# google/forma

Hardware: AMD Instinct MI355X
Metric: frames/sec (sorted+painted, device-resident) + Mpixel-segments/sec (higher is better)
Workload: dtype u64 segments / f64+f32 rasterizer / f32 painter; 1 GPU; paris-like-30k-4k (labelled stand-in: paris-30k.svg is not in the reference checkout); layers=30000, pixel_segments=13757174, frames_in_flight=3

## Files before the change

forma_amd/csrc/api.cpp:

```cpp
#include <new>

#include "ctx.h"

#ifndef FORMA_ARCH
#define FORMA_ARCH "gfx950"
#endif

thread_local KernelTimer* g_ktimer = nullptr;
static inline float* kt_us(forma_hip_ctx* c) { return c->kt_dur_us; }

int fd_fail(forma_hip_ctx* c, int code, const char* what, hipError_t e) {
    if (c) snprintf(c->err, sizeof c->err, "%s%s%s", what, e != hipSuccess ? ": " : "", e != hipSuccess ? hipGetErrorString(e) : "");
    return code;
}

namespace {

inline int fail(forma_hip_ctx* c, int code, const char* what, hipError_t e = hipSuccess) { return fd_fail(c, code, what, e); }
void share_scene(forma_hip_ctx* o);
void invalidate_counts(forma_hip_ctx* o);
inline forma_hip_ctx* last_slot(forma_hip_ctx* ctx) { return ctx->last ? ctx->last : ctx; }
#define HIPCHECK(expr)                                                        \
    do {                                                                      \
        hipError_t _e = (expr);                                               \
// ... 52 lines not shown
    const uint32_t bf_cap = (uint32_t)std::min<size_t>(ctx->block_first.cap / 4, 0xFFFFFFFFu);
    stage_begin(ctx, ST_PREPARE, timing);
    launch_prepare_compact(ctx->stream, src, (uint32_t)n_lines, ctx->cl_idx.as<uint32_t>(), ctx->cl_start.as<uint32_t>(),
                           ctx->block_first.as<uint32_t>(), bf_cap, ctx->prep_scratch.as<uint32_t>(), ctx->info.as<FrameInfo>(), zero);
    stage_end(ctx, ST_PREPARE, timing);
    HIPCHECK(hipGetLastError());
    if (bound_n) return FORMA_OK;
    int rc = read_info(ctx);
    if (rc) return rc;
    const size_t N = ctx->h_info->n_segments;
    ctx->n_seg = N; ctx->n_compact = ctx->h_info->n_compact;
    const size_t need = (N + RAS_TILE - 1) / RAS_TILE + 1;
    if (need > bf_cap) {
        HIPCHECK(ctx->block_first.ensure(need * 4 * 2));
        launch_block_first(ctx->stream, ctx->cl_start.as<uint32_t>(), (uint32_t)ctx->n_compact, (uint32_t)N,
                           ctx->block_first.as<uint32_t>());
    }
    return FORMA_OK;
}

LineSource geometry_source(forma_hip_ctx* ctx, uint32_t width, uint32_t height) {
    LineSource S;
    memset(&S, 0, sizeof S);
    const size_t l0 = ctx->line_ranged ? ctx->line_lo : 0;
    S.x = ctx->x.as<float>() + l0; S.y = ctx->y.as<float>() + l0; S.line_slot = ctx->line_slot.as<uint32_t>() + l0;
    S.geoms = ctx->geoms.as<forma_geom_t>(); S.n_geoms = (uint32_t)ctx->n_geoms;
    S.width = (float)width; S.height = (float)height;
    S.band_lo = -3.0e38f; S.band_hi = 3.0e38f;
    if (ctx->band_row1 > 0) { S.band_lo = (float)(ctx->band_row0 * 16u) - 0.125f; S.band_hi = (float)(ctx->band_row1 * 16u) + 0.125f; }
    return S;
}

int finish_rasterize(forma_hip_ctx* ctx) {
    int rc = read_info(ctx);
    if (rc) return rc;
    uint64_t k_or = (uint64_t)ctx->h_info->key_or | ((uint64_t)ctx->h_info->key_or_hi << 32);
    uint64_t k_and = (uint64_t)ctx->h_info->key_and | ((uint64_t)ctx->h_info->key_and_hi << 32);
    ctx->live44 = (k_or ^ k_and) & 0xFFFFFFFFFFFull;
    ctx->layer_sorted = ctx->h_info->layer_unsorted == 0;
    return FORMA_OK;
}

SortPlan frame_sort_plan(forma_hip_ctx* ctx, uint64_t live44, bool layer_sorted, int digit_bits, bool speculated, bool* biased);
static bool fuse_plan_ok(const forma_hip_ctx* ctx, const SortPlan& plan);

int run_rasterize_frame(forma_hip_ctx* ctx, uint32_t width, uint32_t height, bool timing, bool speculate = false,
                        uint32_t bound_n = 0, const ZeroJobs* zero = nullptr, const forma_hip_ctx::PreZero* cleared = nullptr,
                        bool hist_too = false ) {
    const size_t all_lines = ctx->n_points ? ctx->n_points - 1 : 0;
    const size_t n_lines = ctx->line_ranged ? std::min(ctx->line_hi, all_lines) - std::min(ctx->line_lo, all_lines) : all_lines;
    ctx->n_lines = n_lines;
    ctx->n_seg = 0; ctx->n_compact = 0; ctx->have_unsorted = true; ctx->live44 = 0; ctx->layer_sorted = true;
    ctx->speculated = false; ctx->ras_hist_on = false; ctx->ras_fused = false;
    ctx->pz = forma_hip_ctx::PreZero();
    int rc = reset_info(ctx);
    if (rc) return rc;
    if (n_lines == 0) return FORMA_OK;
    const LineSource S = geometry_source(ctx, width, height);
    if ((rc = run_line_table(ctx, S, n_lines, timing, bound_n, zero))) return rc;
    if (zero && cleared) ctx->pz = *cleared;
    FrameInfo* dinfo = ctx->info.as<FrameInfo>();
    DevCount nc_seg, nc_cmp;
    if (bound_n) {
        nc_seg = DevCount{&dinfo->n_segments, bound_n};
        nc_cmp = DevCount{&dinfo->n_compact, (uint32_t)n_lines};
    } else {
        const size_t N = ctx->n_seg;
        if (N == 0) return FORMA_OK;
        if (N >= (1ull << 30)) return fail(ctx, FORMA_E_CAPACITY, "more than 2^30-1 pixel segments on one device");
        nc_seg = DevCount{nullptr, (uint32_t)N};
        nc_cmp = DevCount{nullptr, (uint32_t)ctx->n_compact};
    }
    HIPCHECK(ctx->seg_u.ensure(((size_t)nc_seg.bound + SEG_PAD) * 8));
    HIPCHECK(ctx->ras_masks.ensure(((size_t)nc_seg.bound / RAS_TILE + 2) * 32));
    RasHist RH;
    memset(&RH, 0, sizeof RH);
    if (hist_too && bound_n && ctx->pred_valid && ctx->pz.sort_p && ctx->pz.sort_p == ctx->sort_counters.p && !ctx->dbg.no_ras_hist) {
        ctx->ras_plan = frame_sort_plan(ctx, ctx->pred_live44, ctx->pred_layer_sorted, ctx->digit_bits, true, nullptr);
        RH = make_ras_hist(ctx->ras_plan, ctx->sort_counters.as<uint32_t>());
        ctx->ras_hist_on = RH.hist != nullptr;
        if (RH.hist && ctx->pz.slice_p && ctx->pz.slice_p == ctx->slice_buf.p && ctx->pz.slice_words >= slice_tab_words(bound_n) &&
            fuse_plan_ok(ctx, ctx->ras_plan)) {
            const SliceSrc SS = make_slice_src(ctx->slice_buf.as<uint32_t>(), bound_n);
            RH.slice_tab = SS.tab; RH.tab_stride = SS.tab_stride;
            ctx->ras_fused = true;
        }
        {
            const SortPlan plain = make_segment_sort_plan(ctx->pred_live44, ctx->pred_layer_sorted, ctx->digit_bits, nullptr, nullptr);
            const SortPlan lay = ctx->pred_layer_sorted ? SortPlan{} : make_sort_plan((ctx->pred_live44 & 0x1FFFFFull) << 20, 20, 41, ctx->digit_bits);
            bool biased = false;
            for (int p = 0; p < ctx->ras_plan.n_passes; p++) biased |= ctx->ras_plan.fmask[p] != 0u;
            RH.track_range = (biased || plain.n_passes > (ctx->pred_layer_sorted ? 0 : lay.n_passes) + 2) ? 1u : 0u;
        }
    }
    stage_begin(ctx, ST_RASTER, timing);
    launch_rasterize(ctx->stream, S, nc_cmp, nc_seg, ctx->cl_idx.as<uint32_t>(), ctx->cl_start.as<uint32_t>(),
                     ctx->block_first.as<uint32_t>(), ctx->seg_u.as<uint64_t>(), dinfo, (int)ctx->band_row0,
                     (int)ctx->band_row1, ctx->ras_masks.as<uint32_t>(), bound_n == 0, &RH);
    ctx->pending_masks = bound_n ? PendingMasks{ctx->ras_masks.as<uint32_t>(), 0u, ctx->ras_hist_on ? 1u : 0u} : PendingMasks{nullptr, 0u, 0u};
    ctx->seg_u_fused = ctx->ras_fused; ctx->fused_w = width; ctx->fused_h = height;
    stage_end(ctx, ST_RASTER, timing);
    HIPCHECK(hipGetLastError());
    ctx->speculated = (speculate || bound_n) && ctx->pred_valid;
    if (ctx->speculated) {
        ctx->live44 = ctx->pred_live44; ctx->layer_sorted = ctx->pred_layer_sorted;
        return FORMA_OK;
    }
    return finish_rasterize(ctx);
}

static uint32_t sort_workgroups(const forma_hip_ctx* ctx, size_t n_keys) {
    if (ctx->dbg.sort_cus >= 0) return (uint32_t)ctx->dbg.sort_cus;
    const forma_hip_ctx* o = ctx->owner ? ctx->owner : ctx;
    const size_t slots = o->slots.size();
    if (ctx->frame_has_dst) return 0u;
    return slots == 3 || (slots == 2 && n_keys >= ((size_t)1 << 22)) ? o->n_cus / 2u : 0u;
}

#ifndef CARRY_HALF_SLICED
#define CARRY_HALF_SLICED 1
#endif
static bool one_frame_in_flight(const forma_hip_ctx* ctx) {
    const forma_hip_ctx* o = ctx->owner ? ctx->owner : ctx;
    return o->slots.size() <= 1;
}
static bool paint_by_strips(const forma_hip_ctx* ctx, uint32_t tiles_painted) {
    if (ctx->dbg.strip_tiles >= 0) return tiles_painted <= (uint32_t)ctx->dbg.strip_tiles;
    return tiles_painted <= paint_strip_tiles(ctx) && !ctx->scene_simple && (uint64_t)ctx->costly_layers * 32u >= ctx->n_orders && one_frame_in_flight(ctx);
}

static bool paint_by_quads(const forma_hip_ctx* ctx, int cache_id, uint32_t runs_bound, uint32_t tiles) {
    if (!ctx->scene_simple || ctx->dbg.no_simple_paint || cache_id >= 0 || ctx->dbg.paint_quad == 0) return false;
    if (ctx->dbg.paint_quad == 2) return true;
    return tiles >= 16u * 8192u && (uint64_t)runs_bound <= 8ull * tiles;
}

static void ban_bias(forma_hip_ctx* ctx) {
    ctx->bias_ban_len = ctx->bias_ban_len ? std::min(ctx->bias_ban_len * 2u, 4096u) : 64u;
    ctx->bias_banned = ctx->bias_ban_len;
}

SortPlan frame_sort_plan(forma_hip_ctx* ctx, uint64_t live44, bool layer_sorted, int digit_bits, bool speculated, bool* biased) {
    const KeyRange* range = speculated && ctx->pred_range.valid && !ctx->bias_banned && !ctx->dbg.no_bias ? &ctx->pred_range : nullptr;
    return make_segment_sort_plan(live44, layer_sorted, digit_bits, range, biased);
}

#ifndef FUSE_MIN_SLICE
#define FUSE_MIN_SLICE 28
#endif
#ifndef FUSE_PROBE
#define FUSE_PROBE 256
#endif
static bool fuse_plan_ok(const forma_hip_ctx* ctx, const SortPlan& plan) {
    if (ctx->dbg.fuse_digit == 0 || ctx->dbg.no_ras_hist || ctx->digit_bits == 4) return false;
    if (ctx->band_row1 > 0 || ctx->line_ranged) return false;
    return plan.n_passes >= 2 && plan.n_passes <= RH_MAX_PASSES && plan.mask[0] <= 255u;
}
static bool fuse_first_digit(forma_hip_ctx* ctx, const SortPlan& plan) {
    if (!fuse_plan_ok(ctx, plan)) return false;
    if (ctx->dbg.fuse_digit == 2 || ctx->pred_slice_len == 0 || ctx->pred_slice_len >= FUSE_MIN_SLICE) return true;
    if (++ctx->fuse_skipped < FUSE_PROBE) return false;
    ctx->fuse_skipped = 0;
    return true;
}

int plan_zero_jobs(forma_hip_ctx* ctx, uint32_t width, uint32_t height, uint32_t sort_n, uint32_t runs_n, ZeroJobs* Z,
                   forma_hip_ctx::PreZero* cleared) {
// ... 1947 lines not shown
```

forma_amd/csrc/common.h:

```cpp
#pragma once
#include <hip/hip_runtime.h>
#include <hip/hip_ext.h>
#include <stdint.h>
#include <stddef.h>

#include "../../include/forma_hip.h"

#define SEG_KEY_SHIFT 20
#define SEG_KEY_BITS  44

#if defined(__HIPCC__)
#define FD __device__ __forceinline__
#else
#define FD inline
#endif

FD int      seg_tile_y(uint64_t v) { return (int)(v >> 53) - 1; }
FD int      seg_tile_x(uint64_t v) { return (int)((v >> 41) & 0xFFFu) - 1; }
FD uint32_t seg_layer(uint64_t v) { return (uint32_t)(v >> 20) & 0x1FFFFFu; }
FD int      seg_lx(uint64_t v) { return (int)(v >> 16) & 0xF; }
FD int      seg_ly(uint64_t v) { return (int)(v >> 12) & 0xF; }
FD int      seg_dam(uint64_t v) { return (int)(v >> 6) & 0x3F; }
FD int      seg_cover(uint64_t v) { return ((int)(v & 0x3F) ^ 0x20) - 0x20; }
FD uint64_t seg_key(uint64_t v) { return v >> SEG_KEY_SHIFT; }
// ... 63 lines not shown
    uint4*   list;
    uint32_t cap;
    uint32_t min_row;
};

struct TileCacheArgs {
    uint2*         tiles;
    uint8_t*       written;
};
#define REF_SPAN 0x80000000u
#define REF_UNCH 0x40000000u
#define REF_IDX  0x3FFFFFFFu

struct DevCount {
    const uint32_t* ptr;
    uint32_t bound;
};
#if defined(__HIPCC__)
__device__ __forceinline__ uint32_t dev_count(DevCount c) { return c.ptr ? min(*c.ptr, c.bound) : c.bound; }
#endif

struct KernelTimer {
    static constexpr int CAP = 96;
    hipEvent_t e0[CAP], e1[CAP];
    const char* name[CAP];
    int stage[CAP];
    int n = 0, made = 0, cur_stage = 0;
    int dropped = 0;
    hipStream_t stream = nullptr;
};
extern thread_local KernelTimer* g_ktimer;
inline bool ktimer_slot(KernelTimer* kt, const char* name, hipEvent_t* e0, hipEvent_t* e1) {
    if (!kt) return false;
    if (kt->n >= KernelTimer::CAP) { kt->dropped++; return false; }
    if (kt->n >= kt->made) {
        if (hipEventCreate(&kt->e0[kt->made]) != hipSuccess) return false;
        if (hipEventCreate(&kt->e1[kt->made]) != hipSuccess) { (void)hipEventDestroy(kt->e0[kt->made]); return false; }
        kt->made++;
    }
    const int i = kt->n++;
    kt->name[i] = name; kt->stage[i] = kt->cur_stage;
    *e0 = kt->e0[i]; *e1 = kt->e1[i];
    return true;
}
#define FORMA_LAUNCH(kern, grid, block, shm, s, ...)                                                        \
    do {                                                                                                    \
        hipEvent_t fl_e0_, fl_e1_;                                                                          \
        if (g_ktimer && g_ktimer->stream == (s) && ktimer_slot(g_ktimer, #kern, &fl_e0_, &fl_e1_))          \
            hipExtLaunchKernelGGL(kern, grid, block, shm, s, fl_e0_, fl_e1_, 0, __VA_ARGS__);               \
        else                                                                                                \
            hipLaunchKernelGGL(kern, grid, block, shm, s, __VA_ARGS__);                                     \
    } while (0)

void launch_prepare_lines(hipStream_t s, const float* x, const float* y, const uint32_t* line_slot, uint32_t n_lines,
                          const forma_geom_t* geoms, uint32_t n_geoms, float width, float height, float band_lo,
                          float band_hi, uint32_t* orders, float* x0, float* y0, float* dx, float* dy, float* a,
                          float* b, float* c, float* d, uint32_t* lengths);
size_t scan_tmp_words(size_t n);
void launch_inclusive_scan_u32(hipStream_t s, uint32_t* data, size_t n, uint32_t* tmp, uint32_t* d_total);
void launch_exclusive_scan_u32(hipStream_t s, uint32_t* data, size_t n, uint32_t* tmp, uint32_t* d_total);
void launch_scan_small_u32(hipStream_t s, uint32_t* data, DevCount n, uint32_t per, uint32_t* d_total);

#define RAS_TILE 2048u
struct PendingMasks { const uint32_t* rec; uint32_t n_fixed; uint32_t has_range; };
struct LineSource {
    const float* x; const float* y; const uint32_t* line_slot; const forma_geom_t* geoms; uint32_t n_geoms;
    float width, height, band_lo, band_hi;
    const uint32_t* sums;
    const uint32_t* orders; const float *x0, *y0, *dx, *dy, *a, *b, *c, *d;
};
size_t prepare_scratch_words(size_t n_lines);
struct ZeroJobs;
void launch_prepare_compact(hipStream_t s, const LineSource& src, uint32_t n_lines, uint32_t* cl_idx, uint32_t* cl_start,
                            uint32_t* block_first, uint32_t bf_cap, uint32_t* scratch, FrameInfo* info,
                            const ZeroJobs* zero );
void launch_line_lengths(hipStream_t s, const LineSource& src, uint32_t n_lines, uint32_t* lens, uint32_t* scratch );
void launch_block_first(hipStream_t s, const uint32_t* cl_start, uint32_t n_compact, uint32_t n_segments,
                        uint32_t* block_first);
#define HS_COPIES  16
#define SORT_BINS  512
#define RH_MAX_PASSES 3
struct RasHist { uint32_t* hist; uint32_t n_passes; uint32_t shift[RH_MAX_PASSES], mask[RH_MAX_PASSES], bias[RH_MAX_PASSES], fmask[RH_MAX_PASSES];
                 uint32_t track_range;
                 uint32_t* slice_tab; uint32_t tab_stride;  };
void launch_rasterize(hipStream_t s, const LineSource& src, DevCount n_compact, DevCount n_segments,
                      const uint32_t* cl_idx, const uint32_t* cl_start, const uint32_t* block_first, uint64_t* out,
                      FrameInfo* info, int band_row0, int band_row1, uint32_t* wg_masks ,
                      bool reduce_now ,
                      const RasHist* hist = nullptr);
void launch_flatten(hipStream_t s, const forma_flatten_tables_t* dev_tables, float* out_x, float* out_y);

#define SORT_MAX_PASSES 12
struct SortPlan {
    int      n_passes;
    int      shift[SORT_MAX_PASSES];
    uint32_t mask[SORT_MAX_PASSES];
    uint32_t bias[SORT_MAX_PASSES];
    uint32_t fmask[SORT_MAX_PASSES];
};
struct KeyRange { uint32_t min_x, max_x, min_y, max_y; bool valid; };
SortPlan make_sort_plan(uint64_t live_mask, int lo_bit, int hi_bit, int digit_bits);
SortPlan make_segment_sort_plan(uint64_t live44, bool layer_sorted, int digit_bits, const KeyRange* range, bool* biased);
size_t sort_scratch_words(size_t n);
size_t sort_zero_words(size_t n, const SortPlan& plan);
const uint32_t* sort_range_words(const uint32_t* scratch);
struct SliceSrc {
    uint32_t* tab; uint32_t tab_stride; uint32_t* first; uint32_t first_cap; uint2* ent; uint32_t ent_cap; };
struct ChunkedSrc { const uint64_t* buckets; uint32_t n_chunks; uint32_t capacity; uint32_t* mask_records; };
uint32_t sort_hist_blocks(size_t n);
const uint64_t* launch_radix_sort(hipStream_t s, const uint64_t* in, uint64_t* a, uint64_t* b, DevCount n,
                                  const SortPlan& plan, int digit_bits, uint32_t* scratch, uint32_t* err,
                                  const ChunkedSrc* chunked = nullptr, FrameInfo* info = nullptr,
                                  bool scratch_is_zero = false ,
                                  bool hist_ready = false ,
                                  uint32_t max_workgroups = 0 ,
                                  const SliceSrc* sliced = nullptr );
RasHist make_ras_hist(const SortPlan& plan, uint32_t* sort_scratch);
#define SLICE_NZ_ROW (SORT_MAX_PASSES - 1)
size_t slice_scratch_words(size_t n);
size_t slice_tab_words(size_t n);
SliceSrc make_slice_src(uint32_t* scratch, size_t n);

#define FORMA_MAX_RANKS 8
struct OwnerBands { uint32_t n; uint32_t edge[FORMA_MAX_RANKS + 1]; };
size_t owner_scratch_words(size_t n);
void launch_owner_bucket(hipStream_t s, const uint64_t* seg, DevCount n, const OwnerBands& B, uint32_t capacity,
                         uint32_t* scratch, uint64_t* send, FrameInfo* info);
void launch_row_histogram(hipStream_t s, const uint64_t* seg, DevCount n, uint32_t* hist );
size_t gather_mask_words(uint32_t n_ranks, uint32_t capacity);
void launch_gather_chunks(hipStream_t s, const uint64_t* recv, uint32_t n_ranks, uint32_t capacity,
                          uint64_t* out, FrameInfo* info, uint32_t* mask_records , bool reduce_now);

struct BlkEdge {
    uint32_t cov[4];
    uint32_t cnt;
    uint32_t has_boundary;
    uint32_t pad[2];
};
size_t runs_scratch_words(size_t n);
size_t runs_blocks(size_t n);
struct RunStyle {
    const uint32_t* layer_sf;
    uint32_t        n_orders;
    const uint8_t*  unchanged;
    uint32_t*       run_lt;
};
#define RUN_LT_OPEN 0x8000u
#define RUN_LT_NEWTILE 0x4000u
struct BlkRuns {
    const TileRecord* rec_sp;
    const uint32_t*   run_lt_sp;
    const uint32_t*   heads;
    const uint32_t*   row_sp;
    uint32_t*         row_base_out;
    uint32_t*         tile_first_run;
    uint32_t*         run_lt_out;
    uint32_t          round_tiles;
};
void launch_runs(hipStream_t s, const uint64_t* sorted, DevCount n, uint32_t tiles_w, uint32_t tiles_h, TileRecord* records,
                 uint32_t rec_cap, uint64_t* run_keys, uint32_t* tile_first_run, BlkEdge* blk_edge,
                 uint32_t* row_tab, uint32_t* scratch, FrameInfo* info, bool verify_plan, uint64_t spec_live44,
                 bool spec_layer_sorted, PendingMasks pm, RunStyle rs, bool tables_are_zero,
                 const uint32_t* range_records ,
                 uint32_t n_range_records ,
                 int what = 3 ,
                 uint32_t* chain_row_base = nullptr ,
                 bool chain_status_is_zero = false ,
// ... 90 lines not shown
```

forma_amd/csrc/debug.h:

```cpp
#pragma once
#include <cstdlib>
#include <cstring>
#include <algorithm>

struct ForMaDebug {
    bool sync = false, global_runsort = false, xgather = false, no_small_carry = false, span_groups = false, no_span_groups = false;
    bool no_packed_copy = false, no_simple_paint = false, force_simple_paint = false, trim_debug = false, force_exchange = false;
    bool xchg_copy = false, no_prezero = false, no_bias = false, no_ras_hist = false, no_cull = false, force_cull = false, no_order = false;
    int carry_slices = 0, digit_bits = 0, poison = -1, poison_frame = -1, strip_tiles = -1, carry_half = 1, paint_quad = 1, order_thr = -1, sort_cus = -1, runs_chain = -1, multi_layout = 0, carry_covl = 1, runs_blk = -1, blk_round = 256, tail_poll = 1, paint_split = 1, split_first = 25, fuse_digit = 1;
};

inline ForMaDebug forma_debug_parse() {
    ForMaDebug d;
    const char* e = getenv("FORMA_HIP_DEBUG");
    if (!e) return d;
    char buf[512];
    strncpy(buf, e, sizeof buf - 1); buf[sizeof buf - 1] = 0;
    char* save = nullptr;
    for (char* tok = strtok_r(buf, ",; ", &save); tok; tok = strtok_r(nullptr, ",; ", &save)) {
        char* val = strchr(tok, '=');
        if (val) *val++ = 0;
        const long v = val ? strtol(val, nullptr, 0) : 0;
#define FD_FLAG(name) if (!strcmp(tok, #name)) { d.name = true; continue; }
        FD_FLAG(sync) FD_FLAG(global_runsort) FD_FLAG(xgather) FD_FLAG(no_small_carry) FD_FLAG(span_groups) FD_FLAG(no_span_groups)
        FD_FLAG(no_cull) FD_FLAG(force_cull) FD_FLAG(no_order) FD_FLAG(no_prezero) FD_FLAG(no_bias) FD_FLAG(no_ras_hist) FD_FLAG(no_packed_copy) FD_FLAG(no_simple_paint) FD_FLAG(force_simple_paint) FD_FLAG(trim_debug) FD_FLAG(force_exchange)
#undef FD_FLAG
        if (!strcmp(tok, "xchg")) { d.xchg_copy = val && !strcmp(val, "copy"); continue; }
        if (!strcmp(tok, "multi_layout")) { d.multi_layout = val && !strcmp(val, "exchange") ? 1 : (val && !strcmp(val, "bands") ? 2 : 0); continue; }
        if (!strcmp(tok, "carry_slices")) { d.carry_slices = (int)v; continue; }
        if (!strcmp(tok, "digit_bits")) { d.digit_bits = (int)v; continue; }
        if (!strcmp(tok, "carry_half")) { d.carry_half = (int)std::max(v, 0L); continue; }
        if (!strcmp(tok, "carry_covl")) { d.carry_covl = (int)std::max(v, 0L); continue; }
        if (!strcmp(tok, "sort_cus")) { d.sort_cus = (int)std::max(v, 0L); continue; }
        if (!strcmp(tok, "order_thr")) { d.order_thr = (int)std::max(v, 0L); continue; }
        if (!strcmp(tok, "paint_quad")) { d.paint_quad = (int)std::max(v, 0L); continue; }
        if (!strcmp(tok, "runs_chain")) { d.runs_chain = (int)std::max(v, 0L); continue; }
        if (!strcmp(tok, "runs_blk")) { d.runs_blk = (int)std::max(v, 0L); continue; }
        if (!strcmp(tok, "blk_round")) { d.blk_round = (int)std::min(std::max(v, 1L), 256L); continue; }
        if (!strcmp(tok, "paint_split")) { d.paint_split = (int)std::min(std::max(v, 0L), 8L); continue; }
        if (!strcmp(tok, "split_first")) { d.split_first = (int)std::min(std::max(v, 1L), 99L); continue; }
        if (!strcmp(tok, "fuse_digit")) { d.fuse_digit = (int)std::min(std::max(v, 0L), 2L); continue; }
        if (!strcmp(tok, "tail_poll")) { d.tail_poll = (int)std::max(v, 0L); continue; }
        if (!strcmp(tok, "strip_tiles")) { d.strip_tiles = (int)std::max(v, 0L); continue; }
        if (!strcmp(tok, "poison")) { d.poison = (int)(v & 0xFF); continue; }
        if (!strcmp(tok, "poison_frame")) { d.poison_frame = (int)(v & 0xFF); continue; }
    }
    return d;
}
```

forma_amd/csrc/lines.hip:

```cpp
#include "common.h"
#include "lookback.h"
#include "radix_rank.h"
#include <string.h>
#ifdef RAS_PROF
__device__ unsigned long long g_ras_prof[64][8];
#define RP_STAMP(i) do { const unsigned long long _t = __builtin_readcyclecounter(); if (threadIdx.x == 0) atomicAdd(&g_ras_prof[blockIdx.x & 63][i], _t - rp_t); rp_t = __builtin_readcyclecounter(); } while (0)
extern "C" int forma_hip_debug_ras_prof(unsigned long long* out8, int reset) {
    static unsigned long long h[64][8];
    if (reset) { for (int c = 0; c < 64; c++) for (int i = 0; i < 8; i++) h[c][i] = 0; return (int)hipMemcpyToSymbol(HIP_SYMBOL(g_ras_prof), h, sizeof h); }
    int rc = (int)hipMemcpyFromSymbol(h, HIP_SYMBOL(g_ras_prof), sizeof h);
    for (int i = 0; i < 8; i++) { out8[i] = 0; for (int c = 0; c < 64; c++) out8[i] += h[c][i]; }
    return rc;
}
#else
#define RP_STAMP(i) do { } while (0)
#endif

#define WAVE 64

__device__ __forceinline__ uint32_t wave_inclusive_scan(uint32_t v) {
    const int lane = threadIdx.x & 63;
#pragma unroll
    for (int d = 1; d < 64; d <<= 1) {
        uint32_t t = __shfl_up(v, d, 64);
// ... 416 lines not shown
}

__device__ __forceinline__ uint64_t rasterize_one(uint32_t order, float lx0, float ly0, float ldx, float ldy, float a,
                                                  float b, float c, float d, double a_ab, double b_ab, double cd_ab,
                                                  uint32_t seg_i) {
    int i = (int)seg_i - (c != 0.0f ? 1 : 0) - (d != 0.0f ? 1 : 0);
    float t0 = fmaxf(find_term(i, a_ab, b_ab, cd_ab, a, b, c, d), 0.0f);
    float t1 = fminf(find_term(i + 1, a_ab, b_ab, cd_ab, a, b, c, d), 1.0f);
    float x0f = fmaf(t0, ldx, lx0), y0f = fmaf(t0, ldy, ly0);
    float x1f = fmaf(t1, ldx, lx0), y1f = fmaf(t1, ldy, ly0);
    int x0s = (int)floorf(x0f + 0.5f), x1s = (int)floorf(x1f + 0.5f);
    int y0s = (int)floorf(y0f + 0.5f), y1s = (int)floorf(y1f + 0.5f);
    int border_x = min(x0s, x1s) >> 4, border_y = min(y0s, y1s) >> 4;
    int tile_x = (int)(int16_t)(border_x >> 4), tile_y = (int)(int16_t)(border_y >> 4);
    uint32_t lx = (uint32_t)border_x & 15u, ly = (uint32_t)border_y & 15u;
    int border = (int)((uint32_t)border_x << 4) + 16;
    uint32_t dam = (uint32_t)(abs(x1s - x0s) + 2 * (border - max(x0s, x1s))) & 0xFFu;
    int cover = (int)(int8_t)(y1s - y0s);
    int ty1 = (int)(int16_t)(tile_y + 1), tx1 = (int)(int16_t)(tile_x + 1);
    uint64_t v = (uint64_t)(ty1 > 0 ? ty1 : 0) & 0x7FFull;
    v = (v << 12) | ((uint64_t)(tx1 > 0 ? tx1 : 0) & 0xFFFull);
    v = (v << 21) | ((uint64_t)order & 0x1FFFFFull);
    v = (v << 4) | lx;
    v = (v << 4) | ly;
    v = (v << 6) | (dam & 0x3Fu);
    v = (v << 6) | ((uint32_t)cover & 0x3Fu);
    return v;
}

__device__ __forceinline__ int round_half_up(float x) { return (int)floorf(x + 0.5f); }
__device__ __forceinline__ float find_term_k(int i, double a_k, double b_k, double cda_k, double cdb_k, float a, float b, float c, float d) {
    const float fi = (float)i;
    const float ja = (float)ceil(fma(b_k, (double)fi, cdb_k));
    const float jb = (float)ceil(fma(a_k, (double)fi, cda_k));
    return fminf(fmaf(a, ja, c), fmaf(b, jb, d));
}
__device__ __forceinline__ uint64_t rasterize_one_k(uint32_t order, float lx0, float ly0, float ldx, float ldy, float a, float b, float c,
                                                    float d, double a_k, double b_k, double cda_k, double cdb_k, int i) {
    float t0 = fmaxf(find_term_k(i, a_k, b_k, cda_k, cdb_k, a, b, c, d), 0.0f);
    float t1 = fminf(find_term_k(i + 1, a_k, b_k, cda_k, cdb_k, a, b, c, d), 1.0f);
    float x0f = fmaf(t0, ldx, lx0), y0f = fmaf(t0, ldy, ly0);
    float x1f = fmaf(t1, ldx, lx0), y1f = fmaf(t1, ldy, ly0);
    int x0s = round_half_up(x0f), x1s = round_half_up(x1f);
    int y0s = round_half_up(y0f), y1s = round_half_up(y1f);
    int border_x = min(x0s, x1s) >> 4, border_y = min(y0s, y1s) >> 4;
    int tile_x = (int)(int16_t)(border_x >> 4), tile_y = (int)(int16_t)(border_y >> 4);
    uint32_t lx = (uint32_t)border_x & 15u, ly = (uint32_t)border_y & 15u;
    int border = (int)((uint32_t)border_x << 4) + 16;
    uint32_t dam = (uint32_t)(abs(x1s - x0s) + 2 * (border - max(x0s, x1s))) & 0xFFu;
    int cover = (int)(int8_t)(y1s - y0s);
    int ty1 = (int)(int16_t)(tile_y + 1), tx1 = (int)(int16_t)(tile_x + 1);
    uint64_t v = (uint64_t)(ty1 > 0 ? ty1 : 0) & 0x7FFull;
    v = (v << 12) | ((uint64_t)(tx1 > 0 ? tx1 : 0) & 0xFFFull);
    v = (v << 21) | ((uint64_t)order & 0x1FFFFFull);
    v = (v << 4) | lx;
    v = (v << 4) | ly;
    v = (v << 6) | (dam & 0x3Fu);
    v = (v << 6) | ((uint32_t)cover & 0x3Fu);
    return v;
}

__device__ __forceinline__ LineP load_line(const LineSource& S, uint32_t li) {
    if (S.sums) {
        LineP L;
        L.order = S.orders[li]; L.x0 = S.x0[li]; L.y0 = S.y0[li]; L.dx = S.dx[li]; L.dy = S.dy[li];
        L.a = S.a[li]; L.b = S.b[li]; L.c = S.c[li]; L.d = S.d[li]; L.len = 1;
        return L;
    }
    return line_params(S.x, S.y, S.line_slot, li, S.geoms, S.n_geoms, S.width, S.height, S.band_lo, S.band_hi);
}

#ifndef RAS_OCC
#define RAS_OCC 6
#endif
struct RasWindow {
    double aab[RAS_WIN], bab[RAS_WIN], cdab[RAS_WIN], cdb[RAS_WIN];
    float x0[RAS_WIN], y0[RAS_WIN], dx[RAS_WIN], dy[RAS_WIN], a[RAS_WIN], b[RAS_WIN], c[RAS_WIN], d[RAS_WIN];
    uint32_t start[RAS_WIN + 1], order[RAS_WIN];
    int ioff[RAS_WIN];
};
union RasLds { RasWindow w; uint64_t stg[RAS_TILE]; };
static_assert(sizeof(uint64_t) * RAS_TILE <= sizeof(RasWindow), "the partition staging lives in the line window");

__device__ __forceinline__ void ras_partition(const uint64_t (&vout)[RAS_PER_THREAD], uint64_t* __restrict__ out, const RasHist& RH,
                                              uint64_t* stg, uint16_t* wc , uint32_t* wsum ,
                                              uint32_t k0, uint32_t k1) {
    constexpr int WAVES = RAS_THREADS / 64, PER_WAVE = 64 * RAS_PER_THREAD;
    static_assert(WAVES * 256 * 2 <= SORT_BINS * 4, "the wave counters live in lh's first row");
    static_assert(RAS_THREADS == 256, "one digit per thread");
    const int tid = threadIdx.x, lane = tid & 63, w = tid >> 6;
    const uint32_t sh = RH.shift[0], mk = RH.mask[0], bs = RH.bias[0];
    const uint32_t nloc = k1 - k0;
#pragma unroll
    for (int q = 0; q < RAS_PER_THREAD; q += 2)
        *reinterpret_cast<ulonglong2*>(&stg[tid * RAS_PER_THREAD + q]) = make_ulonglong2(vout[q], vout[q + 1]);
    __syncthreads();
    uint64_t kk[RAS_PER_THREAD];
    uint32_t rk[RAS_PER_THREAD / 2];
    uint32_t* wcw = reinterpret_cast<uint32_t*>(wc) + w * 128;
#pragma unroll
    for (int j = 0; j < RAS_PER_THREAD; j++) {
        const uint32_t i = w * PER_WAVE + j * 64 + lane;
        kk[j] = stg[i];
        const uint32_t dg = i < nloc ? (((uint32_t)(kk[j] >> sh) - bs) & mk) : mk;
        uint32_t mlo, mhi;
        match_any<8>(dg, mlo, mhi);
        const uint32_t below = lanes_below(mlo, mhi), cnt = (uint32_t)__popc(mlo) + (uint32_t)__popc(mhi);
        const uint32_t hs = (dg & 1u) * 16u;
        if (below == 0) atomicAdd(&wcw[dg >> 1], cnt << hs);
        __builtin_amdgcn_fence(__ATOMIC_RELEASE, "wavefront");
        const uint32_t r = ((wcw[dg >> 1] >> hs) & 0xFFFFu) - cnt + below;
        if (j & 1) rk[j >> 1] |= r << 16; else rk[j >> 1] = r;
    }
    __syncthreads();
    {
        const uint32_t d = (uint32_t)tid;
        uint32_t c[WAVES], tot = 0;
#pragma unroll
        for (int q = 0; q < WAVES; q++) { c[q] = wc[q * 256 + d]; tot += c[q]; }
        uint32_t incl = tot;
#pragma unroll
        for (int o = 1; o < 64; o <<= 1) { const uint32_t v = __shfl_up(incl, o, 64); if (lane >= o) incl += v; }
        if (lane == 63) wsum[w] = incl;
        __syncthreads();
        uint32_t off = incl - tot;
        for (int q = 0; q < w; q++) off += wsum[q];
        uint32_t acc = off;
#pragma unroll
        for (int q = 0; q < WAVES; q++) { wc[q * 256 + d] = (uint16_t)acc; acc += c[q]; }
        if (d == mk) tot -= RAS_TILE - nloc;
        if (tot) {
            RH.slice_tab[(size_t)d * RH.tab_stride + blockIdx.x] = (off << 12) | tot;
            uint32_t* mine = RH.hist + (size_t)(blockIdx.x % HS_COPIES) * (SORT_MAX_PASSES * SORT_BINS);
            atomicAdd(&mine[d], tot);
            atomicAdd(&mine[SLICE_NZ_ROW * SORT_BINS + d], 1u);
        }
    }
    __syncthreads();
#pragma unroll
    for (int j = 0; j < RAS_PER_THREAD; j++) {
        const uint32_t i = w * PER_WAVE + j * 64 + lane;
        const uint32_t dg = i < nloc ? (((uint32_t)(kk[j] >> sh) - bs) & mk) : mk;
        stg[wc[w * 256 + dg] + ((rk[j >> 1] >> ((j & 1) * 16)) & 0xFFFFu)] = kk[j];
    }
    __syncthreads();
#pragma unroll
    for (int q = 0; q < RAS_PER_THREAD; q += 2) {
        const uint32_t i = (uint32_t)q * RAS_THREADS + 2u * tid;
        if (i + 1 < nloc) *reinterpret_cast<ulonglong2*>(out + k0 + i) = *reinterpret_cast<const ulonglong2*>(&stg[i]);
        else if (i < nloc) out[k0 + i] = stg[i];
    }
}

template <bool HIST, bool FUSE = false>
__global__ __launch_bounds__(RAS_THREADS, RAS_OCC) void k_rasterize(LineSource S, DevCount nc_compact, DevCount nc_segments,
                                                           const uint32_t* __restrict__ cl_idx,
                                                           const uint32_t* __restrict__ cl_start,
                                                           const uint32_t* __restrict__ block_first,
                                                           uint64_t* __restrict__ out, FrameInfo* __restrict__ info,
                                                           int band_row0, int band_row1, uint32_t* __restrict__ wg_masks,
                                                           RasHist RH) {
    __shared__ uint32_t lh[HIST ? RH_MAX_PASSES * SORT_BINS : 1];
    __shared__ RasLds lw;
    uint32_t (&w_start)[RAS_WIN + 1] = lw.w.start;
    uint32_t (&w_order)[RAS_WIN] = lw.w.order;
    float (&w_x0)[RAS_WIN] = lw.w.x0; float (&w_y0)[RAS_WIN] = lw.w.y0; float (&w_dx)[RAS_WIN] = lw.w.dx; float (&w_dy)[RAS_WIN] = lw.w.dy;
    float (&w_a)[RAS_WIN] = lw.w.a; float (&w_b)[RAS_WIN] = lw.w.b; float (&w_c)[RAS_WIN] = lw.w.c; float (&w_d)[RAS_WIN] = lw.w.d;
    double (&w_aab)[RAS_WIN] = lw.w.aab; double (&w_bab)[RAS_WIN] = lw.w.bab; double (&w_cdab)[RAS_WIN] = lw.w.cdab; double (&w_cdb)[RAS_WIN] = lw.w.cdb;
    int (&w_ioff)[RAS_WIN] = lw.w.ioff;
    __shared__ uint32_t red[HIST ? (FUSE ? 8 : 7) : 5][RAS_THREADS / 64];
    const int tid = threadIdx.x;
    const uint32_t n_segments = dev_count(nc_segments), n_compact = dev_count(nc_compact);
    const uint32_t bf_lo = block_first[blockIdx.x], bf_hi = block_first[blockIdx.x + 1];
    const uint32_t nblocks = (n_segments + RAS_TILE - 1) / RAS_TILE;
    const uint32_t k0 = blockIdx.x * RAS_TILE;
    if (k0 >= n_segments) return;
    const uint32_t k1 = min(k0 + RAS_TILE, n_segments);
#ifdef RAS_PROF
    unsigned long long rp_t = __builtin_readcyclecounter();
    if (tid == 0) atomicAdd(&g_ras_prof[blockIdx.x & 63][7], 1ull);
#endif
    const uint32_t lo = bf_lo;
    const uint32_t hi = blockIdx.x + 1 < nblocks ? bf_hi : n_compact - 1;
    uint32_t k_or = 0, k_or_hi = 0, k_and = 0xFFFFFFFFu, k_and_hi = 0xFFFFFFFFu, unsorted = 0;
    const uint32_t kt = k0 + tid * RAS_PER_THREAD;
    uint64_t vout[RAS_PER_THREAD];
#pragma unroll
    for (int q = 0; q < RAS_PER_THREAD; q++) vout[q] = 0;
    if (HIST) for (uint32_t i = tid; i < RH.n_passes * SORT_BINS; i += RAS_THREADS) lh[i] = 0;

    for (uint32_t c0 = lo; c0 <= hi; c0 += RAS_WIN) {
        const uint32_t cnt = min((uint32_t)RAS_WIN, hi - c0 + 1);
        if (c0 != lo) __syncthreads();
        for (uint32_t j = tid; j < cnt; j += RAS_THREADS) {
            const uint32_t cidx = c0 + j;
            LineP L;
// ... 253 lines not shown
```

Measured before the change: 3144 frames/s.

## Rank rasterizer partition keys by digit runs instead of per-key wave matching

In the fused rasterize-partition step, each lane now computes digits for its own contiguous keys and finds runs of equal digits. When a wave has at most 64 runs, it ranks whole runs with ballot/mbcnt prefix sums and a small LDS table, replacing eight per-key match_any plus LDS-atomic rounds. Ranks are exchanged through a wave-local LDS buffer, and the first block barrier becomes wave-level syncs. A debug flag and the many-runs case fall back to the old per-key path; the extra LDS traffic and more complex bookkeeping are the cost.

```diff
diff --git a/forma_amd/csrc/api.cpp b/forma_amd/csrc/api.cpp
--- a/forma_amd/csrc/api.cpp
+++ b/forma_amd/csrc/api.cpp
@@ -158,7 +158,7 @@
         if (RH.hist && ctx->pz.slice_p && ctx->pz.slice_p == ctx->slice_buf.p && ctx->pz.slice_words >= slice_tab_words(bound_n) &&
             fuse_plan_ok(ctx, ctx->ras_plan)) {
             const SliceSrc SS = make_slice_src(ctx->slice_buf.as<uint32_t>(), bound_n);
-            RH.slice_tab = SS.tab; RH.tab_stride = SS.tab_stride;
+            RH.slice_tab = SS.tab; RH.tab_stride = SS.tab_stride; RH.per_key = ctx->dbg.rank_keys ? 1u : 0u;
             ctx->ras_fused = true;
         }
         {
diff --git a/forma_amd/csrc/common.h b/forma_amd/csrc/common.h
--- a/forma_amd/csrc/common.h
+++ b/forma_amd/csrc/common.h
@@ -169,7 +169,8 @@
 #define RH_MAX_PASSES 3
 struct RasHist { uint32_t* hist; uint32_t n_passes; uint32_t shift[RH_MAX_PASSES], mask[RH_MAX_PASSES], bias[RH_MAX_PASSES], fmask[RH_MAX_PASSES];
                  uint32_t track_range;
-                 uint32_t* slice_tab; uint32_t tab_stride;  };
+                 uint32_t* slice_tab; uint32_t tab_stride;
+                 uint32_t per_key;  };
 void launch_rasterize(hipStream_t s, const LineSource& src, DevCount n_compact, DevCount n_segments,
                       const uint32_t* cl_idx, const uint32_t* cl_start, const uint32_t* block_first, uint64_t* out,
                       FrameInfo* info, int band_row0, int band_row1, uint32_t* wg_masks ,
diff --git a/forma_amd/csrc/debug.h b/forma_amd/csrc/debug.h
--- a/forma_amd/csrc/debug.h
+++ b/forma_amd/csrc/debug.h
@@ -6,7 +6,7 @@
 struct ForMaDebug {
     bool sync = false, global_runsort = false, xgather = false, no_small_carry = false, span_groups = false, no_span_groups = false;
     bool no_packed_copy = false, no_simple_paint = false, force_simple_paint = false, trim_debug = false, force_exchange = false;
-    bool xchg_copy = false, no_prezero = false, no_bias = false, no_ras_hist = false, no_cull = false, force_cull = false, no_order = false;
+    bool xchg_copy = false, no_prezero = false, no_bias = false, no_ras_hist = false, rank_keys = false, no_cull = false, force_cull = false, no_order = false;
     int carry_slices = 0, digit_bits = 0, poison = -1, poison_frame = -1, strip_tiles = -1, carry_half = 1, paint_quad = 1, order_thr = -1, sort_cus = -1, runs_chain = -1, multi_layout = 0, carry_covl = 1, runs_blk = -1, blk_round = 256, tail_poll = 1, paint_split = 1, split_first = 25, fuse_digit = 1;
 };
 
@@ -23,7 +23,7 @@
         const long v = val ? strtol(val, nullptr, 0) : 0;
 #define FD_FLAG(name) if (!strcmp(tok, #name)) { d.name = true; continue; }
         FD_FLAG(sync) FD_FLAG(global_runsort) FD_FLAG(xgather) FD_FLAG(no_small_carry) FD_FLAG(span_groups) FD_FLAG(no_span_groups)
-        FD_FLAG(no_cull) FD_FLAG(force_cull) FD_FLAG(no_order) FD_FLAG(no_prezero) FD_FLAG(no_bias) FD_FLAG(no_ras_hist) FD_FLAG(no_packed_copy) FD_FLAG(no_simple_paint) FD_FLAG(force_simple_paint) FD_FLAG(trim_debug) FD_FLAG(force_exchange)
+        FD_FLAG(no_cull) FD_FLAG(force_cull) FD_FLAG(no_order) FD_FLAG(no_prezero) FD_FLAG(no_bias) FD_FLAG(no_ras_hist) FD_FLAG(rank_keys) FD_FLAG(no_packed_copy) FD_FLAG(no_simple_paint) FD_FLAG(force_simple_paint) FD_FLAG(trim_debug) FD_FLAG(force_exchange)
 #undef FD_FLAG
         if (!strcmp(tok, "xchg")) { d.xchg_copy = val && !strcmp(val, "copy"); continue; }
         if (!strcmp(tok, "multi_layout")) { d.multi_layout = val && !strcmp(val, "exchange") ? 1 : (val && !strcmp(val, "bands") ? 2 : 0); continue; }
diff --git a/forma_amd/csrc/lines.hip b/forma_amd/csrc/lines.hip
--- a/forma_amd/csrc/lines.hip
+++ b/forma_amd/csrc/lines.hip
@@ -522,36 +522,110 @@
 union RasLds { RasWindow w; uint64_t stg[RAS_TILE]; };
 static_assert(sizeof(uint64_t) * RAS_TILE <= sizeof(RasWindow), "the partition staging lives in the line window");
 
+__device__ __forceinline__ void wave_lds_sync() {
+    __builtin_amdgcn_fence(__ATOMIC_RELEASE, "wavefront");
+    __builtin_amdgcn_wave_barrier();
+    __builtin_amdgcn_fence(__ATOMIC_ACQUIRE, "wavefront");
+}
+
 __device__ __forceinline__ void ras_partition(const uint64_t (&vout)[RAS_PER_THREAD], uint64_t* __restrict__ out, const RasHist& RH,
                                               uint64_t* stg, uint16_t* wc , uint32_t* wsum ,
                                               uint32_t k0, uint32_t k1) {
     constexpr int WAVES = RAS_THREADS / 64, PER_WAVE = 64 * RAS_PER_THREAD;
     static_assert(WAVES * 256 * 2 <= SORT_BINS * 4, "the wave counters live in lh's first row");
     static_assert(RAS_THREADS == 256, "one digit per thread");
+    static_assert(RAS_PER_THREAD == 8, "a lane's keys: one row of the rank buffer's layout");
     const int tid = threadIdx.x, lane = tid & 63, w = tid >> 6;
     const uint32_t sh = RH.shift[0], mk = RH.mask[0], bs = RH.bias[0];
     const uint32_t nloc = k1 - k0;
+    uint64_t* ws = stg + w * PER_WAVE;
 #pragma unroll
     for (int q = 0; q < RAS_PER_THREAD; q += 2)
         *reinterpret_cast<ulonglong2*>(&stg[tid * RAS_PER_THREAD + q]) = make_ulonglong2(vout[q], vout[q + 1]);
-    __syncthreads();
+    uint32_t dq[RAS_PER_THREAD];
+#pragma unroll
+    for (int q = 0; q < RAS_PER_THREAD; q++) dq[q] = ((uint32_t)(vout[q] >> sh) - bs) & mk;
+    if (nloc < RAS_TILE) {
+#pragma unroll
+        for (int q = 0; q < RAS_PER_THREAD; q++) if ((uint32_t)(tid * RAS_PER_THREAD + q) >= nloc) dq[q] = mk;
+    }
+    wave_lds_sync();
     uint64_t kk[RAS_PER_THREAD];
+#pragma unroll
+    for (int j = 0; j < RAS_PER_THREAD; j++) kk[j] = ws[j * 64 + lane];
+    wave_lds_sync();
+    uint16_t* rb = reinterpret_cast<uint16_t*>(ws);
+    uint32_t sm = 0;
+#pragma unroll
+    for (int q = 1; q < RAS_PER_THREAD; q++) sm |= (dq[q - 1] != dq[q] ? 1u : 0u) << q;
+    const uint32_t prev = (uint32_t)__shfl_up((int)dq[RAS_PER_THREAD - 1], 1, 64);
+    if (lane == 0 || dq[0] != prev) sm |= 1u;
+    const uint32_t ns = (uint32_t)__popc(sm);
+    uint32_t r0 = 0, nruns = 0;
+#pragma unroll
+    for (int b = 3; b >= 0; b--) {
+        const uint64_t bal = __ballot((ns >> b) & 1u);
+        r0 = lanes_below((uint32_t)bal, (uint32_t)(bal >> 32)) + r0 + r0;
+        nruns = (uint32_t)__popcll(bal) + nruns + nruns;
+    }
+    if (!RH.per_key && nruns <= 64u) {
+        uint32_t* tab = reinterpret_cast<uint32_t*>(ws) + 256;
+        const uint32_t p0 = (uint32_t)lane * RAS_PER_THREAD;
+        {
+            uint32_t r = r0;
+#pragma unroll
+            for (int q = 0; q < RAS_PER_THREAD; q++)
+                if ((sm >> q) & 1u) { tab[r] = (p0 + q) | (dq[q] << 16); r++; }
+        }
+        if (lane == 0) tab[nruns] = PER_WAVE;
+        wave_lds_sync();
+        const uint32_t e = tab[lane], en = tab[lane + 1];
+        const bool act = (uint32_t)lane < nruns;
+        const uint32_t st = e & 0xFFFFu, dr = act ? e >> 16 : 0u, lr = act ? (en & 0xFFFFu) - st : 0u;
+        uint32_t mlo, mhi;
+        match_any<8>(dr, mlo, mhi);
+        const uint32_t below = lanes_below(mlo, mhi);
+        uint32_t B = 0;
+        if (__ballot(act && below != 0u)) {
+#pragma unroll
+            for (int b = 8; b >= 0; b--) {
+                const uint64_t bal = __ballot((lr >> b) & 1u);
+                B = __builtin_amdgcn_mbcnt_hi(mhi & (uint32_t)(bal >> 32), __builtin_amdgcn_mbcnt_lo(mlo & (uint32_t)bal, B + B));
+            }
+        }
+        const uint64_t am = nruns >= 64u ? ~0ull : ((1ull << nruns) - 1ull);
+        const uint32_t cnt_act = (uint32_t)__popc(mlo & (uint32_t)am) + (uint32_t)__popc(mhi & (uint32_t)(am >> 32));
+        if (act && below + 1u == cnt_act) wc[w * 256 + dr] = (uint16_t)(B + lr);
+        wave_lds_sync();
+        tab[lane] = B - st;
+        wave_lds_sync();
+        const uint32_t bi = ((uint32_t)(lane >> 4) * 64u + (uint32_t)(lane & 7) * 8u) * 2u + ((uint32_t)(lane >> 3) & 1u);
+        uint32_t r = r0 - 1u;
+#pragma unroll
+        for (int q = 0; q < RAS_PER_THREAD; q++) {
+            r += (sm >> q) & 1u;
+            rb[bi + 2 * q] = (uint16_t)(tab[r] + p0 + q);
+        }
+    } else {
+        uint32_t* wcw = reinterpret_cast<uint32_t*>(wc) + w * 128;
+#pragma unroll 1
+        for (int j = 0; j < RAS_PER_THREAD; j++) {
+            const uint32_t i = w * PER_WAVE + j * 64 + lane;
+            const uint32_t dg = i < nloc ? (((uint32_t)(ws[j * 64 + lane] >> sh) - bs) & mk) : mk;
+            uint32_t mlo, mhi;
+            match_any<8>(dg, mlo, mhi);
+            const uint32_t below = lanes_below(mlo, mhi), cnt = (uint32_t)__popc(mlo) + (uint32_t)__popc(mhi);
+            const uint32_t hs = (dg & 1u) * 16u;
+            if (below == 0) atomicAdd(&wcw[dg >> 1], cnt << hs);
+            __builtin_amdgcn_fence(__ATOMIC_RELEASE, "wavefront");
+            const uint32_t r = ((wcw[dg >> 1] >> hs) & 0xFFFFu) - cnt + below;
+            rb[((j >> 1) * 64 + lane) * 2 + (j & 1)] = (uint16_t)r;
+        }
+    }
+    wave_lds_sync();
     uint32_t rk[RAS_PER_THREAD / 2];
-    uint32_t* wcw = reinterpret_cast<uint32_t*>(wc) + w * 128;
-#pragma unroll
-    for (int j = 0; j < RAS_PER_THREAD; j++) {
-        const uint32_t i = w * PER_WAVE + j * 64 + lane;
-        kk[j] = stg[i];
-        const uint32_t dg = i < nloc ? (((uint32_t)(kk[j] >> sh) - bs) & mk) : mk;
-        uint32_t mlo, mhi;
-        match_any<8>(dg, mlo, mhi);
-        const uint32_t below = lanes_below(mlo, mhi), cnt = (uint32_t)__popc(mlo) + (uint32_t)__popc(mhi);
-        const uint32_t hs = (dg & 1u) * 16u;
-        if (below == 0) atomicAdd(&wcw[dg >> 1], cnt << hs);
-        __builtin_amdgcn_fence(__ATOMIC_RELEASE, "wavefront");
-        const uint32_t r = ((wcw[dg >> 1] >> hs) & 0xFFFFu) - cnt + below;
-        if (j & 1) rk[j >> 1] |= r << 16; else rk[j >> 1] = r;
-    }
+#pragma unroll
+    for (int jp = 0; jp < RAS_PER_THREAD / 2; jp++) rk[jp] = reinterpret_cast<const uint32_t*>(rb)[jp * 64 + lane];
     __syncthreads();
     {
         const uint32_t d = (uint32_t)tid;
```

Measured after the change: 3168 frames/s (median of 6 runs). Within noise of the previous version (+0.8%).
